# guenthermi/postgres-word2vec

Hardware: AMD Instinct MI355X
Metric: batched IVFADC kNN queries/sec (k=5) + recall@5, 3Mx300d (higher is better)
Workload: dtype f32; 1 GPU; IVFADC batch (ivfadc_batch_search generalised to nprobe), 3000000x300d, C=1000, m=12, K=1024, nprobe=10, k=5, batch=1024 queries per GPU, replicated index, queries sharded by rank; N=3000000, d=300, C=1000, m=12, K=1024, nprobe=10, k=5, batch_per_gpu=1024, parallelism=dp1, world_size=1, backend=none (single GPU), batches_in_flight=4

## Files before the change

postgres-word2vec_amd/csrc/fused5.h:

```cpp
#pragma once
#include <hip/hip_runtime.h>
#include <stdint.h>

#include "refine.h"
#include "coarse.h"
#include "scan_tail5.h"

namespace freddy {

static constexpr int SCAN5_G = 16;

__host__ __device__ __forceinline__ constexpr int filt5_bias(int p, int m) { return FILT5_VMAX + (p < 32768 - FILT5_VMAX * m ? 1 : 0); }
__device__ __forceinline__ uint32_t lane_byte4() {
  uint32_t x;
  asm volatile("v_mbcnt_lo_u32_b32 %0, -1, 0\n\tv_mbcnt_hi_u32_b32 %0, -1, %0\n\tv_lshlrev_b32 %0, 2, %0" : "=v"(x));
  return x;
}
typedef short s2v __attribute__((ext_vector_type(2)));
__device__ __forceinline__ uint32_t pk_add_i16(uint32_t x, uint32_t y) {
  return __builtin_bit_cast(uint32_t, __builtin_bit_cast(s2v, x) + __builtin_bit_cast(s2v, y));
}

template <int S, int QT>
__device__ __forceinline__ void query_codebook5_body(const float* __restrict__ queries, const float* __restrict__ cbT,
                                                     const float* __restrict__ cmax, float* __restrict__ qn,
                                                     float* __restrict__ qscale, uint32_t* __restrict__ qc,
                                                     int Q, int d, int m, int K, int bx, int by, unsigned char* smem,
                                                     uint32_t* __restrict__ qc8 = nullptr) {
  static_assert(QT == 16, "one 16-lane group per query");
  constexpr int SP = (S + 3) & ~3;
  float (*qs)[SP] = reinterpret_cast<float (*)[SP]>(smem);
  float* inv_s = reinterpret_cast<float*>(smem + QT * SP * 4);
  const int tid = threadIdx.x, p = bx, q0 = by * QT;
  static_assert(S <= 32 && SP % 4 == 0, "one k-step of v_mfma_f32_16x16x32_f16 covers a position");
  ch8v bh[8], bl[8];
  auto load_b = [&](int g) {
    const ch8v* src = reinterpret_cast<const ch8v*>(cbT) + ((size_t)p * 8 + g) * (CBF_GROUP_HALVES / 8) + (tid & 63);
#pragma unroll
    for (int t = 0; t < 8; ++t) { bh[t] = src[(size_t)t * 128]; bl[t] = src[(size_t)t * 128 + 64]; }
  };
  load_b((tid >> 6) * 2);
  const int ecb = reinterpret_cast<const int*>(cbT)[cbf_exp_offset(m) + p];
  for (int i = tid; i < QT * SP; i += 256) {
    const int qi = i / SP, j = i - qi * SP;
    qs[qi][j] = (j < S && q0 + qi < Q) ? queries[(size_t)(q0 + qi) * d + p * S + j] : 0.0f;
  }
  {
    const int qi = tid >> 4, pp = tid & 15, q = q0 + qi;
    float best = 0.0f;
    if (pp < m && q < Q) {
      float n2 = 0.0f;
      for (int j = 0; j < S; ++j) { const float v = queries[(size_t)q * d + pp * S + j]; n2 = __builtin_fmaf(v, v, n2); }
      const float nrm = __builtin_sqrtf(n2) * (1.0f + 1e-5f);
      if (p == 0) qn[(size_t)q * m + pp] = nrm;
      best = 2.0f * nrm * cmax[pp];
    }
#pragma unroll
    for (int o = 8; o > 0; o >>= 1) best = fmaxf(best, __shfl_xor(best, o, 64));
    if (pp == 0) {
      const float sc = q < Q ? best * (1.0f / (float)FILT5_VMAX) * (1.0f + 1e-6f) : 0.0f;
      inv_s[qi] = (sc > 0.0f && sc < 1e30f) ? 1.0f / sc : 0.0f;
      if (p == 0 && q < Q) qscale[q] = sc;
    }
  }
  {
    typedef float f4v __attribute__((ext_vector_type(4)));
    __syncthreads();
    const int wave = tid >> 6, lane = tid & 63, col = lane & 15, kq = lane >> 4;
    const int nq = (Q - q0 < QT) ? Q - q0 : QT;
    ch8v ah, al;
    int eq = 0;
    {
      f4v x0 = f4v{0.0f, 0.0f, 0.0f, 0.0f}, x1 = x0;
      if (8 * kq < SP) x0 = *reinterpret_cast<const f4v*>(&qs[col][8 * kq]);
      if (8 * kq + 4 < SP) x1 = *reinterpret_cast<const f4v*>(&qs[col][8 * kq + 4]);
      const float x[8] = {x0.x, x0.y, x0.z, x0.w, x1.x, x1.y, x1.z, x1.w};
      float am = 0.0f;
#pragma unroll
      for (int j = 0; j < 8; ++j) am = fmaxf(am, __builtin_fabsf(x[j]));
      am = fmaxf(am, __shfl_xor(am, 16, 64));
      am = fmaxf(am, __shfl_xor(am, 32, 64));
      if (am > 0.0f && am < 3e38f) { (void)__builtin_frexpf(am, &eq); eq = CBF_EXP - eq; }
#pragma unroll
      for (int j = 0; j < 8; ++j) {
        const float v = __builtin_ldexpf(x[j], eq);
        const _Float16 hh = (_Float16)v;
        ah[j] = hh;
        al[j] = (_Float16)(v - (float)hh);
      }
    }
    int unscale[4];
#pragma unroll
    for (int reg = 0; reg < 4; ++reg) unscale[reg] = -(__shfl(eq, 4 * kq + reg, 64) + ecb);
// ... 218 lines not shown
    };

    long long pt[8] = {0, 0, 0, 0, 0, 0, 0, 0}, pc = 0;
    auto tick = [&](int slot) { if constexpr (PROF) { const long long t = clock64(); pt[slot] += t - pc; pc = t; } };
    if constexpr (PROF) pc = clock64();
    int nq = (__builtin_amdgcn_readfirstlane(dsc[1]) + 7) >> 3;
    const int g0 = half * 8;
    int qid[8], nqid[8];
#pragma unroll
    for (int u = 0; u < 8; ++u) {
      qid[u] = __builtin_amdgcn_readfirstlane(dsc[24 + g0 + u]);
      nqid[u] = qid[u];
    }
    float rtv[RMAX];
    auto fetch_row_terms = [&](const int32_t* rc) {
      const int b0 = __builtin_amdgcn_readfirstlane(rc[3]), nbk = __builtin_amdgcn_readfirstlane(rc[4]);
#pragma unroll
      for (int r = 0; r < RMAX; ++r) {
        const int bl = r * NG + wave;
        rtv[r] = a.rterm[(size_t)(uint32_t)(b0 + (bl < nbk - 1 ? bl : nbk - 1)) * 64u + (uint32_t)lane];
      }
    };
    auto stash_row_terms = [&]() {
#pragma unroll
      for (int r = 0; r < RMAX; ++r) rt_s[(r * NG + wave) * 64 + lane] = rtv[r];
    };
    fetch_row_terms(dsc);
    stash_row_terms();
    issue(0, 0, qid, nq);
    issue(1, 1, qid, nq);
    emit(0, slab, nq);
    issue(0, 2, qid, nq);
    lds_barrier();
    for (;;) {
      const int nb = cur ^ 1;
      const int ngid = __builtin_amdgcn_readfirstlane(gidq[(ei + 1) & 1]);
      const bool have_next = ngid < n_work;
      int gid2 = 0;
      int next_nq = 0;
      int32_t rr0 = 0;
      uint32_t run0 = 0u, run1 = 0u;
#pragma unroll
      for (int j = 0; j < NP; ++j) {
        if (j == 1 && tid < REC_DW) {
          if (tid == 0) gidq[ei & 1] = gid2;
          dsc[nb * REC_DW + tid] = rr0;
          if (wave == 0 && lane == 6) dsc[nb * REC_DW + 6] = have_next ? 1 : -1;
        }
        if (j == NP - 3) {
          const int ncnt = have_next ? __builtin_amdgcn_readfirstlane(dsc[nb * REC_DW + 1]) : 0;
          next_nq = (ncnt + 7) >> 3;
#pragma unroll
          for (int u = 0; u < 8; ++u)
            nqid[u] = !have_next ? qid[u] : __builtin_amdgcn_readfirstlane(dsc[nb * REC_DW + 24 + g0 + u]);
        }
        const int set = (j + 1) & 1;
        if (j + 1 < NP) emit(set, slab + (uint32_t)((j + 1) & 1) * BUFB, nq);
        else emit(set, slab, next_nq);
        if (j + 3 < NP) issue(set, j + 3, qid, nq);
        else issue(set, j + 3 - NP, nqid, next_nq);
        if (j == 2) fetch_row_terms(dsc + (have_next ? nb : cur) * REC_DW);
        if (j == NP - 1 && a.tau_run) {
          const int32_t* rc = dsc + cur * REC_DW;
          const int cn = __builtin_amdgcn_readfirstlane(rc[1]);
          run0 = wave < cn ? a.tau_run[(uint32_t)rc[24 + wave]] : 0u;
          run1 = wave + NG < cn ? a.tau_run[(uint32_t)rc[24 + wave + NG]] : 0u;
        }
        if (j == 0 && tid < REC_DW && have_next) rr0 = a.records[(size_t)ngid * REC_DW + tid];
        if (j == 0 && tid == 0) {
          if (extra && (gidq[2] != 0 || !have_next)) {
            gid2 = 0x7fffffff;
          } else if (extra && __hip_atomic_load(a.elastic + EL_PENDING, FREDDY_RLX_AGENT) > 0) {
            gid2 = 0x7fffffff;
            gidq[2] = 1;
            __hip_atomic_fetch_add(a.elastic + EL_YIELDED, 1, FREDDY_RLX_AGENT);
          } else {
            gid2 = n_own + atomicAdd(a.work_counter, 1);
          }
        }
        tick(0);
        lds_barrier();
        tick(1);
      }
      if (!(a.fence & 4)) {
        const int32_t* rec = dsc + cur * REC_DW;
        const int cnt = __builtin_amdgcn_readfirstlane(rec[1]);
        const int i0 = wave, i1 = wave + NG;
        if (i0 < cnt) {
          uint32_t c0 = colmin[i0 * 64 + lane], c1 = colmin[i1 * 64 + lane];
          wave_sort32_x2(c0, c1);
          uint32_t t0 = __shfl(c0, a.Lt - 1, 64), t1 = __shfl(c1, a.Lt - 1, 64);
          if (lane == 0) {
            if (a.tau_run) {
              auto lower = [&](uint32_t t, int i, uint32_t inv) -> uint32_t {
                return running_bound5(a.tau_run, (uint32_t)rec[24 + i], t, __int_as_float(rec[144 + i]), __int_as_float(rec[160 + i]), inv);
              };
              t0 = lower(t0, i0, run0);
              if (i1 < cnt) t1 = lower(t1, i1, run1);
            }
            thr_s[i0] = a.keep_all ? 0x7f800000u : widen_threshold5(t0, __int_as_float(rec[56 + i0]));
            thr_s[i1] = a.keep_all ? 0x7f800000u : widen_threshold5(t1, __int_as_float(rec[56 + i1]));
          }
          colmin[i0 * 64 + lane] = 0xffffffffu;
          colmin[i1 * 64 + lane] = 0xffffffffu;
        }
      }
      lds_barrier();
      stash_row_terms();
      lds_barrier();
      tick(3);
      if constexpr (PROF) pt[7] += 1;
      if (!have_next) break;
      cur = nb;
      ++ei;
      nq = next_nq;
#pragma unroll
      for (int u = 0; u < 8; ++u) qid[u] = nqid[u];
    }
    if (ELASTIC && tid == 0) __hip_atomic_fetch_sub(a.elastic + EL_ACTIVE, 1, FREDDY_RLX_AGENT);
    if (PROF && a.prof && tid == 0) {
      for (int i = 0; i < 8; ++i) if (i != 2 && i != 4 && i != 5) a.prof[(size_t)blockIdx.x * 8 + i] = pt[i];
      a.prof[(size_t)blockIdx.x * 8 + 6] = wall_clock64();
    }
  } else {
    const int gw = wave - SPEC2_NB;
    uint32_t acc[G / 2][RMAX];
    uint32_t cwa[RMAX], cwb[RMAX];
    constexpr int NPRE = 2;
    uint32_t cpre[NPRE] = {};
    auto prefetch_first_codes = [&](const int32_t* rc) {
      const int b0 = __builtin_amdgcn_readfirstlane(rc[3]), nbk = __builtin_amdgcn_readfirstlane(rc[4]);
      const uint32_t l4 = lane_byte4();
#pragma unroll
      for (int r = 0; r < NPRE; ++r) {
        const int bl = r * NG + gw;
        const uint32_t blk = (uint32_t)(b0 + (bl < nbk - 1 ? bl : nbk - 1));
        const char* rowp = U8 ? reinterpret_cast<const char*>(a.packed8) + (size_t)(blk * (uint32_t)(M / 4)) * 256u
                              : reinterpret_cast<const char*>(a.packed) + (size_t)(blk * (uint32_t)(M / 2)) * 256u;
        cpre[r] = *reinterpret_cast<const uint32_t*>(rowp + l4);
      }
    };
    prefetch_first_codes(dsc);
    lds_barrier();
    long long gt[3] = {0, 0, 0}, gc = 0;
    auto gtick = [&](int slot) { if constexpr (PROF) { const long long t = clock64(); if (slot >= 0) gt[slot] += t - gc; gc = t; } };
    for (;;) {
      gtick(-1);
      const int32_t* rec = dsc + cur * REC_DW;
      const int cnt = __builtin_amdgcn_readfirstlane(rec[1]);
      const int chunk = __builtin_amdgcn_readfirstlane(rec[2]);
      const int blk0 = __builtin_amdgcn_readfirstlane(rec[3]);
      const int nblk = __builtin_amdgcn_readfirstlane(rec[4]);
      const int nrows = __builtin_amdgcn_readfirstlane(rec[5]);
      const int nq = (cnt + 7) >> 3;
      const int nb = cur ^ 1;
      const int rl_wave = (nblk - gw + NG - 1) / NG < 0 ? 0 : (nblk - gw + NG - 1) / NG;
      auto row_block = [&](int r) {
        const int bl = r * NG + gw;
        return (uint32_t)(blk0 + (bl < nblk - 1 ? bl : nblk - 1));
      };
      auto main_loop = [&](auto nqc, auto rlc) {
        constexpr int NQ = decltype(nqc)::value, RL = decltype(rlc)::value;
        auto load_codes = [&](uint32_t (&cw)[RMAX], int pair) {
          const uint32_t l4 = lane_byte4();
#pragma unroll
          for (int r = 0; r < RL; ++r) {
            const char* rowp = U8 ? reinterpret_cast<const char*>(a.packed8) + (size_t)((row_block(r) * (uint32_t)(M / 4) + (uint32_t)(pair >> 1)) * 256u)
                                  : reinterpret_cast<const char*>(a.packed) + (size_t)((row_block(r) * (uint32_t)(M / 2) + (uint32_t)pair) * 256u);
            cw[r] = *reinterpret_cast<const uint32_t*>(rowp + l4);
          }
        };
        auto gather = [&](const uint32_t (&cw)[RMAX], int j) {
          constexpr int DEPTH = NQ == 1 ? 4 : 2;
          u4 va[DEPTH][2][NQ];
          uint32_t bb = (uint32_t)(j & 1) * BUFB;
          asm volatile("" : "+s"(bb));
          auto issue_row = [&](int r) {
            const uint32_t a0 = (U8 ? ((j & 1) ? ((cw[r] >> 12) & 0xff0u) : ((cw[r] << 4) & 0xff0u)) : ((cw[r] << 4) & 0x3ff0u)) + bb;
            const uint32_t a1 = (U8 ? ((j & 1) ? ((cw[r] >> 20) & 0xff0u) : ((cw[r] >> 4) & 0xff0u)) : ((cw[r] >> 12) & 0x3ff0u)) + bb;
#pragma unroll
            for (int q = 0; q < NQ; ++q) va[r % DEPTH][0][q] = *reinterpret_cast<const u4*>(slab + a0 + (uint32_t)q * HALFB);
#pragma unroll
            for (int q = 0; q < NQ; ++q) va[r % DEPTH][1][q] = *reinterpret_cast<const u4*>(slab + a1 + POSB + (uint32_t)q * HALFB);
          };
#pragma unroll
          for (int r = 0; r < DEPTH - 1; ++r) if (r < RL) issue_row(r);
#pragma unroll
          for (int r = 0; r < RL; ++r) {
            if (r + DEPTH - 1 < RL) issue_row(r + DEPTH - 1);
#pragma unroll
            for (int q = 0; q < NQ; ++q) {
              const u4 x = va[r % DEPTH][0][q], y = va[r % DEPTH][1][q];
              acc[q * 4 + 0][r] = acc[q * 4 + 0][r] + x.x + y.x;
              acc[q * 4 + 1][r] = acc[q * 4 + 1][r] + x.y + y.y;
              acc[q * 4 + 2][r] = acc[q * 4 + 2][r] + x.z + y.z;
              acc[q * 4 + 3][r] = acc[q * 4 + 3][r] + x.w + y.w;
            }
            if (r + 1 < RL) __builtin_amdgcn_sched_barrier(0);
          }
        };
#pragma unroll
        for (int h = 0; h < G / 2; ++h)
#pragma unroll
          for (int r = 0; r < RMAX; ++r) acc[h][r] = 0u;
        load_codes(cwa, 0);
#pragma unroll
        for (int r = 0; r < NPRE; ++r) if (r < RL) cwa[r] = cpre[r];
        load_codes(cwb, 1);
#pragma unroll
        for (int j = 0; j < NP; ++j) {
          if (!(a.fence & 2)) {
            if (j & 1) gather(cwb, j); else gather(cwa, j);
          }
          __builtin_amdgcn_sched_barrier(0);
          if (j + 2 < NP && !(a.fence & 64)) {
            if (j & 1) load_codes(cwb, j + 2); else load_codes(cwa, j + 2);
          }
          if (j + 1 < NP) lds_barrier();
        }
      };
      dispatch_nq_rl(nq, rl_wave, main_loop);
#define SCAN_TAIL5_FENCE a.fence
#define SCAN_TAIL5_PART 1
#include "scan_tail5.inc"
      gtick(0);
#define SCAN_TAIL5_PART 2
#include "scan_tail5.inc"
      gtick(1);
      lds_barrier();
      lds_barrier();
      gtick(-1);
#define SCAN_TAIL5_PART 3
#include "scan_tail5.inc"
#undef SCAN_TAIL5_FENCE
      gtick(2);
      const int next_ok = __builtin_amdgcn_readfirstlane(dsc[nb * REC_DW + 6]);
      if (next_ok > 0) prefetch_first_codes(dsc + nb * REC_DW);
      lds_barrier();
      if (next_ok < 0) break;
      cur = nb;
    }
    if (PROF && a.prof && gw == 0 && lane == 0) {
      a.prof[(size_t)blockIdx.x * 8 + 2] = gt[0];
      a.prof[(size_t)blockIdx.x * 8 + 4] = gt[1];
      a.prof[(size_t)blockIdx.x * 8 + 5] = gt[2];
    }
  }
}

template <int M, bool FULLK, bool CAND, bool PROF = false, bool U8 = false>
__global__ __launch_bounds__(SPEC2_T) void ivf_filter5_kernel(FilterArgs a) {
  ivf_filter5_body<M, FULLK, CAND, PROF, U8, false>(a);
}
template <int M, bool FULLK, bool CAND, bool U8 = false>
__global__ __launch_bounds__(SPEC2_T) void ivf_filter5_elastic_kernel(FilterArgs a) {
  ivf_filter5_body<M, FULLK, CAND, false, U8, true>(a);
}

}
```

postgres-word2vec_amd/csrc/ivfadc.hip:

```cpp
#include "internal.h"

#include <functional>

#include "kernels.h"
#include "scan_common.h"
#include "fused3.h"
#include "fused5.h"
#include "fused8.h"
#include "one.h"
#include "sparse5.h"
#include "coarse.h"
#include "multi.h"
#include "io_kernels.h"
#include "bigk.h"
#include "ivf_host.h"
#include "query_ids.h"

static void (*scan_kernel(bool m12, int V, bool floor))(ScanArgs) {
  void (*k)(ScanArgs) = nullptr;
  if (floor) return V != 16 ? nullptr : m12 ? &adc_scan_kernel<12, 16, true> : &adc_scan_kernel<0, 16, true>;
  with_V(V, [&](auto v) { k = m12 ? &adc_scan_kernel<12, decltype(v)::value> : &adc_scan_kernel<0, decltype(v)::value>; });
  return k;
}
static void (*filter_kernel(bool whole, bool u8, bool k1024, bool counts_rows, bool prof, bool elastic = false))(FilterArgs) {
// ... 165 lines not shown
    else if (r.approx)
      hipLaunchKernelGGL(coarse_approx_kernel, dim3(Cpad / 128, (Q + COARSE_TQ - 1) / COARSE_TQ), dim3(256),
                         (size_t)(COARSE_TQ * (ix->dp + 4) + 128) * sizeof(float), s, r.d_q, ix->coarseP, ix->cn2,
                         ws->w_distT.as<float>(), ws->w_qn2.as<float>(), Q, Cpad, d, ix->dp, za, tile_min, C);
    else if (r.tiled)
      hipLaunchKernelGGL((coarse_tile_kernel<2, 16>), dim3(Cpad / 32, (Q + 63) / 64), dim3(256), 0, s, r.d_q, ix->coarseT,
                         ws->w_distT.as<float>(), Q, Cpad, d, za);
    else if (small_zero)
      hipLaunchKernelGGL((coarse_small_kernel<50>), dim3(Cpad / 64, Q), dim3(64), 0, s, r.d_q, ix->coarseT, ws->w_distT.as<float>(), Q, Cpad, d, za);
    else
      hipLaunchKernelGGL((coarse_dist_kernel<16>), dim3(Cpad / WG, (Q + 15) / 16), dim3(WG), (size_t)d * 16 * sizeof(float), s, r.d_q,
                         ix->coarseT, ws->w_distT.as<float>(), Q, Cpad, d);
  });
  HIP_TRY(hipGetLastError());
  return 0;
}

static int ivf_plan(IvfRun& r, PlanArgs& pa) {
  Workspace* ws = r.ws;
  freddy_gpu_index* ix = r.ix;
  hipStream_t s = r.s;
  const int C = ix->C, W = r.W;
  pa = plan_items(r, C);
  pa.dist = ws->w_distT.as<float>(); pa.active = r.active; pa.list_off = ix->list_off;
  pa.used = ws->w_used.as<uint32_t>(); pa.Cpad = ix->Cpad; pa.used_words = (C + 31) / 32;
  pa.cell_count = r.fused ? ws->w_cellcnt.as<int32_t>() : nullptr;
  pa.cell_items = r.fused ? ws->w_sorted.as<int32_t>() : nullptr; pa.cell_cap = r.n_active;
  pa.cell_limit = r.cell_limit;
  const int n_items = r.n_active * W;
  if (r.fused && !(r.zeroed && r.first())) {
    HIP_TRY(hipMemsetAsync(ws->w_cellcnt.p, 0, sizeof(int32_t) * (size_t)C * 2, s));
    HIP_TRY(hipMemsetAsync(ws->w_surv_cnt.p, 0, sizeof(int32_t) * surv_regions(r, (size_t)n_items), s));
  }
  const int PV = pick_V(2 * W);
  const size_t plan_lds = (size_t)(64 + 64 * PV) * sizeof(u64) + (size_t)W * 8;
  if (r.approx) {
    Plan2Args g;
    g.p = pa; g.queries = r.d_q; g.coarse = ix->coarse; g.qn2 = ws->w_qn2.as<float>(); g.item_dist = pa.item_dist;
    g.violations = ix->viol; g.cmax = ix->cmax; g.d = ix->d; g.refine_all = (ix->tune.check_brackets & 2) ? 1 : 0; g.prof = nullptr;
    g.tmin = (r.first() && ix->Cpad > COARSE_MAX_CPAD && ws->w_tmin.p) ? ws->w_tmin.as<float>() : nullptr;
    timed_launch(ix, s, "probe_plan", [&] {
      if (ix->Cpad <= COARSE_MAX_CPAD && r.share > 1) hipLaunchKernelGGL((probe_plan2_kernel<0, false, 1>), dim3(r.n_active), dim3(64), 0, s, g);
      else if (ix->Cpad <= COARSE_MAX_CPAD) hipLaunchKernelGGL((probe_plan2_kernel<0, false>), dim3(r.n_active), dim3(64 * PLAN2_NW), 0, s, g);
      else hipLaunchKernelGGL((probe_plan2_kernel<0, true>), dim3(r.n_active), dim3(64 * PLAN2_NW), 0, s, g);
    });
  } else
  timed_launch(ix, s, "probe_plan", [&] {
    with_V(PV, [&](auto v) { hipLaunchKernelGGL((probe_plan_kernel<decltype(v)::value>), dim3(r.n_active), dim3(64), plan_lds, s, pa); });
  });
  HIP_TRY(hipGetLastError());
  if (!(r.zeroed && r.first())) HIP_TRY(hipMemsetAsync(ws->w_cand.p, 0, sizeof(int32_t) * 2 * r.Q, s));
  return 0;
}

int ivf_work_table(IvfRun& r, WorkTable& wt) {
  Workspace* ws = r.ws;
  freddy_gpu_index* ix = r.ix;
  hipStream_t s = r.s;
  const int n_items = r.n_active * r.W;
  wt = work_counters(ws, ((size_t)n_items / MULTI_G + (size_t)ix->C + 1) * r.upi);
  int32_t* base = ws->w_groups.as<int32_t>();
  wt.group_cell = base; wt.group_first = base + wt.max_groups; wt.group_cnt = base + 2 * wt.max_groups;
  const int sparse_max = r.scan_kernel != 5 ? 0
                         : ix->tune.sparse_items < 0 ? -ix->tune.sparse_items
                         : sparse_by_itself(ix->n_cus, n_items, ix->C) ? ix->tune.sparse_items : 0;
  wt.sp_cap = sparse_max > 0 ? (size_t)n_items * r.upi : 0;
  wt.sp_cell = base + 3 * wt.max_groups; wt.sp_first = wt.sp_cell + wt.sp_cap; wt.sp_chunk = wt.sp_first + wt.sp_cap;
  timed_launch(ix, s, "work_table", [&] {
    hipLaunchKernelGGL(work_table_kernel, dim3(1), dim3(1024), 0, s, ws->w_cellcnt.as<int32_t>(), ix->C, r.n_active, r.scan_kernel == 5 ? SCAN5_G : r.scan_kernel == 2 ? MULTI_G : SPEC2_G, ix->blk_off,
                       wt.group_cell, wt.group_first, wt.group_cnt, wt.n_groups, r.scan_kernel == 5 ? 2 : 0,
                       sparse_max, wt.sp_cell, wt.sp_first, wt.sp_chunk, wt.n_sparse, sparse_max >= 2 ? 1 : 0);
  });
  wt.sp_pairs = sparse_max >= 2;
  HIP_TRY(hipGetLastError());
  if (!(r.zeroed && r.first())) HIP_TRY(hipMemsetAsync(wt.work_counter, 0, 2 * sizeof(int32_t), s));
  return 0;
}

static int scan_prof_buffer(freddy_gpu_index* ix, Workspace* ws, long long** prof, uint32_t* fence = nullptr) {
  *prof = nullptr;
#ifdef FREDDY_LAB
  if (fence) *fence = (uint32_t)ix->tune.scan_fence;
  if (!ix->tune.scan_prof) return 0;
  if (ws->w_prof.ensure(sizeof(long long) * 8 * 1024)) return fail(FREDDY_E_NOMEM, "profile buffer");
  *prof = ws->w_prof.as<long long>();
#endif
  (void)ix; (void)ws; (void)fence;
  return 0;
}

#ifdef FREDDY_LAB
static int scan_prof_print(freddy_gpu_index* ix, hipStream_t s, const long long* prof, unsigned n_persist) {
  std::vector<long long> h(8 * (size_t)n_persist);
  HIP_TRY(hipStreamSynchronize(s));
  HIP_TRY(hipMemcpy(h.data(), prof, sizeof(long long) * h.size(), hipMemcpyDeviceToHost));
  double sum[8] = {0}; long long mx_end = 0, mn_end = -1; double ent = 0;
  for (unsigned b = 0; b < n_persist; ++b) {
    for (int i = 0; i < 6; ++i) sum[i] += (double)h[b * 8 + i];
    ent += (double)h[b * 8 + 7];
    mx_end = std::max(mx_end, h[b * 8 + 6]);
    mn_end = mn_end < 0 ? h[b * 8 + 6] : std::min(mn_end, h[b * 8 + 6]);
  }
  fprintf(stderr, "[scan prof] wgs=%u entries=%.0f  builder cycles/entry: builds=%.0f barrier-wait=%.0f tail=%.0f | gatherer wave 0 (fused5.h): main=%.0f colmin=%.0f S2=%.0f | workgroups ran dry over %.1f us\n",
          n_persist, ent, sum[0] / ent, sum[1] / ent, sum[3] / ent, sum[2] / ent, sum[4] / ent, sum[5] / ent, (mx_end - mn_end) / 100.0);
  (void)ix;
  return 0;
}
static int filter_prof_print(freddy_gpu_index* ix, hipStream_t s, const FilterArgs& fl, bool whole, unsigned n_persist) {
  if (!fl.prof || fl.cand_count || !(whole || fl.K == 1024)) return 0;
  if (!whole) return scan_prof_print(ix, s, fl.prof, n_persist);
  std::vector<long long> h(8 * (size_t)n_persist);
  HIP_TRY(hipStreamSynchronize(s));
  HIP_TRY(hipMemcpy(h.data(), fl.prof, sizeof(long long) * h.size(), hipMemcpyDeviceToHost));
  double sum[8] = {0}, life_max = 0, life_min = 1e30;
  for (unsigned b = 0; b < n_persist; ++b) {
    for (int i = 0; i < 8; ++i) sum[i] += (double)h[b * 8 + i];
    life_max = std::max(life_max, (double)h[b * 8 + 7]); life_min = std::min(life_min, (double)h[b * 8 + 7]);
  }
  int32_t ng = 0;
  HIP_TRY(hipMemcpy(&ng, fl.n_groups, 4, hipMemcpyDeviceToHost));
  const double e = std::max(1, ng);
  fprintf(stderr, "[scan8 prof] wgs=%u entries=%d  gatherer wave 0 cycles/entry (slots 0-5): gather=%.0f B1=%.0f colmin=%.0f B2=%.0f S1=%.0f B3+S2+B4=%.0f | per workgroup: prologue (slot 6) %.0f, stages (0-5) %.0f, life (slot 7) mean %.0f min %.0f max %.0f\n",
          n_persist, ng, sum[0] / e, sum[1] / e, sum[2] / e, sum[3] / e, sum[4] / e, sum[5] / e, sum[6] / n_persist,
          (sum[0] + sum[1] + sum[2] + sum[3] + sum[4] + sum[5]) / n_persist, sum[7] / n_persist, life_min, life_max);
  return 0;
}
#endif

int ivf_scan_filter(IvfRun& r, const PlanArgs& pa, const WorkTable& wt) {
  Workspace* ws = r.ws;
  freddy_gpu_index* ix = r.ix;
  hipStream_t s = r.s;
  const int K = ix->K;
  const QueryTable qt = query_table(ws, ix, r.Q);
  const unsigned n_own = filter_scan_own(ix->n_cus, r.share, ix->tune.reserve_cus, wt.max_groups);
  const bool u8 = ix->packed8 && ix->tune.codes_u8 != 0 && ix->K <= 256;
  const bool whole = u8 && qt.qc8;
  bool elastic = ix->tune.scan_elastic > 0 && r.share > 1 && !r.records_ready && !whole && ix->elastic != nullptr;
#ifdef FREDDY_LAB
  if (ix->tune.scan_prof) elastic = false;
#endif
  const int cap = filter_scan_cap(ix->n_cus, ix->tune.scan_elastic_reserve, ix->tune.reserve_cus, r.share);
  const unsigned n_persist = filter_scan_persist(elastic, n_own, cap, wt.max_groups);
  if (!r.records_ready) {
    if (ws->w_records.ensure(sizeof(int32_t) * REC_DW * wt.max_groups)) return fail(FREDDY_E_NOMEM, "workspace allocation failed");
    RecordArgs ra;
    ra.group_cell = wt.group_cell; ra.group_first = wt.group_first; ra.group_cnt = wt.group_cnt; ra.n_groups = wt.n_groups;
    ra.sorted_item = ws->w_sorted.as<int32_t>(); ra.item_query = pa.item_query; ra.blk_off = ix->blk_off; ra.list_off = ix->list_off;
    ra.item_dist = pa.item_dist; ra.qn = qt.qn; ra.qscale = qt.qscale; ra.pmax = ix->pmax;
    ra.records = ws->w_records.as<int32_t>(); ra.sentinel = r.sentinel;
    ra.elastic = elastic ? ix->elastic : nullptr; ra.n_announce = (int)n_own;
    timed_launch(ix, s, "entry_records", [&] {
      hipLaunchKernelGGL((entry_record5_kernel<12>), dim3((unsigned)((wt.max_groups + 3) / 4)), dim3(256), 0, s, ra);
    });
    HIP_TRY(hipGetLastError());
  }
  FilterArgs fl;
  fl.qc = qt.qc; fl.qc8 = qt.qc8; fl.rterm = ix->rterm; fl.records = ws->w_records.as<int32_t>(); fl.n_groups = wt.n_groups;
  fl.work_counter = wt.work_counter; fl.packed = ix->packed; fl.surv = ws->w_surv.as<u64>(); fl.surv_count = ws->w_surv_cnt.as<int32_t>();
  fl.cand_count = rows_counter(r);
  fl.K = K; fl.L = r.L; fl.Lt = r.Lt; fl.upi = r.upi; fl.sentinel = r.sentinel; fl.keep_all = (ix->tune.check_brackets & 1) ? 1 : 0; fl.fence = 0;
  fl.tau_run = r.running_bound ? ws->w_cand.as<uint32_t>() + r.Q : nullptr;
  if (int rc = scan_prof_buffer(ix, ws, &fl.prof, &fl.fence)) return rc;
  fl.elastic = elastic ? ix->elastic : nullptr; fl.n_own = (int)n_own; fl.cap = cap; fl.elastic_yield = ix->tune.scan_elastic;
  const size_t desc_off = whole ? (size_t)scan8_slab_bytes(12) : (size_t)4 * SCAN5_G * 2 * K;
  const size_t flds = desc_off + 4096 + 64 + (2 * REC_DW + 4) * sizeof(int32_t) + 4096 * sizeof(float);
  fl.desc_offset = (uint32_t)desc_off;
  fl.packed8 = u8 ? ix->packed8 : nullptr;
  const auto filter = filter_kernel(whole, u8, K == 1024, fl.cand_count != nullptr, fl.prof != nullptr, elastic);
  if (!filter) return fail(FREDDY_E_ARG, "internal: no filter scan for this shape");
  timed_launch(ix, s, "ivf_filter", [&] { hipLaunchKernelGGL(filter, dim3(n_persist), dim3(SPEC2_T), flds, s, fl); });
  HIP_TRY(hipGetLastError());
  if (wt.sp_cap > 0) {
    SparseArgs sp;
    sp.qc = qt.qc; sp.qscale = qt.qscale; sp.qn = qt.qn; sp.pmax = ix->pmax; sp.rterm = ix->rterm; sp.packed = ix->packed;
    sp.blk_off = ix->blk_off; sp.list_off = ix->list_off; sp.sorted_item = ws->w_sorted.as<int32_t>(); sp.item_query = pa.item_query;
    sp.item_dist = pa.item_dist; sp.sp_cell = wt.sp_cell; sp.sp_first = wt.sp_first; sp.sp_chunk = wt.sp_chunk;
    sp.n_units = wt.n_sparse; sp.work_counter = wt.sp_counter; sp.surv = fl.surv; sp.surv_count = fl.surv_count; sp.packed8 = fl.packed8;
    sp.cand_count = fl.cand_count; sp.K = K; sp.L = r.L; sp.Lt = r.Lt; sp.upi = r.upi; sp.sentinel = r.sentinel; sp.keep_all = fl.keep_all; sp.tau_run = fl.tau_run;
    const unsigned sp_grid = sparse_grid(ix->n_cus, r.share, ix->tune.reserve_cus, wt.sp_cap, wt.sp_pairs);
    const auto sparse = sparse_kernel(wt.sp_pairs, u8, fl.cand_count != nullptr);
    timed_launch(ix, s, "sparse_items", [&] { hipLaunchKernelGGL(sparse, dim3(sp_grid), dim3(256), 0, s, sp); });
    HIP_TRY(hipGetLastError());
  }
#ifdef FREDDY_LAB
  if (int rc = filter_prof_print(ix, s, fl, whole, n_persist)) return rc;
#endif

  MergeRefineArgs mr;
  mr.surv = fl.surv; mr.surv_count = fl.surv_count; mr.active = r.active; mr.round_rows = pa.round_rows;
  mr.item_cell = pa.item_cell; mr.queries = r.d_q; mr.coarse = ix->coarse; mr.cbR = ix->cbR;
  mr.qn = qt.qn; mr.pmax = ix->pmax; mr.qscale5 = qt.qscale; mr.packed = ix->packed; mr.pos = ix->pos; mr.blk_cell = ix->blk_cell;
  mr.cand_count = fl.cand_count; mr.violations = ix->viol; mr.out_ids = r.d_out_ids; mr.out_dist = r.d_out_dist;
  mr.found = ws->w_found.as<int32_t>(); mr.next_active = r.next; mr.n_next = ws->w_cnt.as<int32_t>();
  mr.status = r.d_status;
  mr.n_active = r.n_active; mr.W = r.W; mr.upi = r.upi; mr.L = r.L; mr.k = r.k; mr.found_rule = r.found_rule;
  mr.first_round = r.first() ? 1 : 0; mr.K = K; mr.d = ix->d; mr.sentinel = r.sentinel;
  mr.refine_all = (ix->tune.check_brackets & 1) ? 1 : 0; mr.fence = 0;
  mr.slices = 0; mr.part = nullptr;
  if (r.merge_slices > 0) {
    const int SL = r.merge_slices;
    if (ws->w_part.ensure(sizeof(u64) * (size_t)r.n_active * SL * r.L)) return fail(FREDDY_E_NOMEM, "workspace allocation failed");
    mr.slices = SL; mr.part = ws->w_part.as<u64>(); mr.W = r.W / SL; mr.n_active = r.n_active * SL;
    timed_launch(ix, s, "merge_refine", [&] {
      hipLaunchKernelGGL((merge_refine_kernel<25, 12, 12, true, true>), dim3(r.n_active * SL), dim3(768), 0, s, mr);
    });
    HIP_TRY(hipGetLastError());
    return launch_merge(ix, s, merge_args_flat(mr.part, r.n_active, SL, r.L, r.k, r.sentinel, nullptr, r.d_out_ids, r.d_out_dist));
  }
  timed_launch(ix, s, "merge_refine", [&] {
    const bool many_regions = (size_t)r.W * r.upi * FUSED_NW > 256;
    if (!many_regions && r.share > 1)
      hipLaunchKernelGGL((merge_refine_kernel<25, 12, 1>), dim3(r.n_active), dim3(64), 0, s, mr);
    else if (many_regions && r.n_active <= 256)
      hipLaunchKernelGGL((merge_refine_kernel<25, 12, 12, true>), dim3(r.n_active), dim3(768), 0, s, mr);
    else if (many_regions)
      hipLaunchKernelGGL((merge_refine_kernel<25, 12, 4, true>), dim3(r.n_active), dim3(256), 0, s, mr);
    else
      hipLaunchKernelGGL((merge_refine_kernel<25, 12, 4>), dim3(r.n_active), dim3(256), 0, s, mr);
  });
  HIP_TRY(hipGetLastError());
  return 0;
}

static int launch_merge_surv(const IvfRun& r, const PlanArgs& pa, const u64* surv, const int32_t* surv_count, const int32_t* cand_count) {
  MergeSurvArgs ms;
  ms.surv = surv; ms.surv_count = surv_count; ms.active = r.active; ms.round_rows = pa.round_rows;
  ms.cand_count = cand_count; ms.out_ids = r.d_out_ids; ms.out_dist = r.d_out_dist;
  ms.found = r.ws->w_found.as<int32_t>(); ms.next_active = r.next; ms.n_next = r.ws->w_cnt.as<int32_t>();
  ms.status = r.d_status;
  ms.n_active = r.n_active; ms.W = r.W; ms.upi = r.upi; ms.L = r.L; ms.k = r.k; ms.found_rule = r.found_rule;
  ms.first_round = r.first() ? 1 : 0; ms.sentinel = r.sentinel;
  timed_launch(r.ix, r.s, "merge_surv", [&] { hipLaunchKernelGGL(merge_surv_kernel, dim3(r.n_active), dim3(64), 0, r.s, ms); });
  HIP_TRY(hipGetLastError());
  return 0;
}

static int ivf_scan_exact(IvfRun& r, const PlanArgs& pa, const WorkTable& wt) {
  Workspace* ws = r.ws;
  freddy_gpu_index* ix = r.ix;
  hipStream_t s = r.s;
  const int K = ix->K;
  FusedArgs fa;
  fa.resid = nullptr; fa.item_query = pa.item_query; fa.queries = r.d_q; fa.coarse = ix->coarse;
  fa.sorted_item = ws->w_sorted.as<int32_t>(); fa.group_cell = wt.group_cell; fa.group_first = wt.group_first;
  fa.group_cnt = wt.group_cnt; fa.n_groups = wt.n_groups; fa.work_counter = wt.work_counter;
// ... 482 lines not shown
```

postgres-word2vec_amd/csrc/scan_tail5.inc:

```
#if SCAN_TAIL5_PART == 1
float base[RMAX];
const int last_blk = nrows > 0 ? (nrows - 1) >> 6 : -1;
const int rs2 = (last_blk >= 0 && (last_blk % NG) == gw && (nrows & 63)) ? last_blk / NG : -1;
const bool live_lane = lane < (nrows & 63);
{
#pragma unroll
  for (int r = 0; r < RMAX; ++r) {
    base[r] = rt_s[(r * NG + gw) * 64 + lane];
    if (r >= rl_wave || (r == rs2 && !live_lane)) base[r] = __uint_as_float(0x7f800000u);
  }
}
#pragma unroll
for (int h = 0; h < G / 2; ++h)
#pragma unroll
  for (int r = 0; r < RMAX; ++r) acc[h][r] ^= 0x80008000u;
#elif SCAN_TAIL5_PART == 2
auto sval = [&](int g, int r, float sc) -> float {
  const uint32_t w = acc[g >> 1][r];
  const int v = (g & 1) ? ((int32_t)w >> 16) : ((int32_t)(w << 16) >> 16);
  return __builtin_fmaf(sc, (float)v, base[r]);
};
const int gi = lane & 15;
const float p_sc = __int_as_float(rec[128 + gi]);
uint32_t live8 = 0u;
#pragma unroll
for (int r = 0; r < RMAX; ++r)
  if (r < rl_wave && !(r == rs2 && !live_lane)) live8 |= 1u << r;
float best[G];
uint32_t sec16[G / 2];
uint32_t apack[2] = {0u, 0u};
#pragma unroll
for (int g = 0; g < G; ++g) best[g] = __uint_as_float(0x7f800000u);
#pragma unroll
for (int i = 0; i < G / 2; ++i) sec16[i] = 0x7f807f80u;
if (!(SCAN_TAIL5_FENCE & 4)) {
#pragma unroll
  for (int g = 0; g < G; ++g) {
    if (g < cnt) {
      const float sc = __int_as_float(__builtin_amdgcn_readlane(__float_as_int(p_sc), g));
      float b1 = __uint_as_float(0x7f800000u), b2 = __uint_as_float(0x7f800000u);
      uint32_t ar = 0u;
#pragma unroll
      for (int r = 0; r < RMAX; ++r) {
        const float sv = sval(g, r, sc);
        b2 = __builtin_amdgcn_fmed3f(b1, b2, sv);
        ar = sv < b1 ? (uint32_t)r : ar;
        b1 = fminf(b1, sv);
      }
      best[g] = b1;
      {
        const uint32_t bb = __float_as_uint(b2);
        const uint32_t dn = ((bb >> 31) ? bb + 0xffffu : bb) >> 16;
        sec16[g >> 1] = (g & 1) ? ((sec16[g >> 1] & 0x0000ffffu) | (dn << 16)) : ((sec16[g >> 1] & 0xffff0000u) | dn);
      }
      asm volatile("" : "+v"(ar));
      apack[g >> 3] |= ar << (3 * (g & 7));
      if (rl_wave > 0) atomicMin(colmin + g * 64 + lane, float_key(b1));
    }
  }
}
#elif SCAN_TAIL5_PART == 3
if (!(SCAN_TAIL5_FENCE & 4)) {
  const float p_thr = __uint_as_float(thr_s[gi]);
  const int p_it = rec[8 + gi];
  const float p_shift = __int_as_float(rec[72 + gi]);
  const float p_off = __int_as_float(rec[40 + gi]);
  const uint32_t p_lo = (uint32_t)rec[88 + gi], p_hi = (uint32_t)rec[104 + gi];
  const int p_q = rec[24 + gi];
  const int p_reg = (p_it * a.upi + chunk) * NG + gw;
  int cntv = 0;
#pragma unroll
  for (int g = 0; g < G; ++g) {
    if (g < cnt) {
      const float thr = __int_as_float(__builtin_amdgcn_readlane(__float_as_int(p_thr), g));
      const float off = __int_as_float(__builtin_amdgcn_readlane(__float_as_int(p_off), g));
      const float shift = __int_as_float(__builtin_amdgcn_readlane(__float_as_int(p_shift), g));
      const uint32_t region = (uint32_t)__builtin_amdgcn_readlane(p_reg, g);
      u64* dst = a.surv + (size_t)region * (size_t)(RMAX * 64);
      int run = 0;
      if constexpr (!CAND) {
       const float second = __uint_as_float((g & 1) ? (sec16[g >> 1] & 0xffff0000u) : (sec16[g >> 1] << 16));
       const u64 multi = __ballot(!(second > thr));
       if (__builtin_expect(multi == 0ull, 1)) {
        const bool pass = !(best[g] > thr);
        const u64 mask = __ballot(pass);
        if (pass) {
          const uint32_t r = (apack[g >> 3] >> (3 * (g & 7))) & 7u;
          const float dlo = fmaxf(0.0f, (best[g] + off) - shift);
          const uint32_t loc = ((uint32_t)(blk0 + gw) + r * (uint32_t)NG) * 64u + (uint32_t)lane;
          dst[lanes_below(mask)] = surv_key5(dlo, loc);
        }
        run = __popcll(mask);
       } else {
        const float sc = __int_as_float(__builtin_amdgcn_readlane(__float_as_int(p_sc), g));
        uint32_t m8 = 0u;
#pragma unroll
        for (int r = RMAX - 1; r >= 0; --r) m8 = m8 + m8 + (!(sval(g, r, sc) > thr) ? 1u : 0u);
        m8 &= live8;
        if ((SCAN_TAIL5_FENCE & 128) == 0 && __ballot(m8 != 0u) != 0ull) {
#pragma unroll
          for (int r = 0; r < RMAX; ++r) {
            const bool pass = (m8 >> r) & 1u;
            const u64 mask = __ballot(pass);
            if (mask != 0ull) {
              if (pass) {
                const float dlo = fmaxf(0.0f, (sval(g, r, sc) + off) - shift);
                const uint32_t loc = (uint32_t)(blk0 + r * NG + gw) * 64u + (uint32_t)lane;
                dst[run + lanes_below(mask)] = surv_key5(dlo, loc);
              }
              run += __popcll(mask);
            }
          }
        }
       }
      } else {
        const uint32_t lo_b = (uint32_t)__builtin_amdgcn_readlane((int)p_lo, g);
        const uint32_t hi_b = (uint32_t)__builtin_amdgcn_readlane((int)p_hi, g);
        const float sc = __int_as_float(__builtin_amdgcn_readlane(__float_as_int(p_sc), g));
        int accepted = 0;
#pragma unroll
        for (int r = 0; r < RMAX; ++r) {
          if (r >= rl_wave) break;
          const float sv = sval(g, r, sc);
          const uint32_t sb = __float_as_uint(sv + off);
          const bool live = (live8 >> r) & 1u;
          accepted += __popcll(__ballot(live && sb < lo_b));
          const bool amb = sb >= lo_b && sb < hi_b;
          const bool pass = live && (!(sv > thr) || amb);
          const u64 mask = __ballot(pass);
          if (mask != 0ull) {
            if (pass) {
              const float dlo = fmaxf(0.0f, __uint_as_float(sb) - shift);
              const uint32_t loc = ((uint32_t)(blk0 + r * NG + gw) * 64u + (uint32_t)lane) | (amb ? 0x80000000u : 0u);
              dst[run + lanes_below(mask)] = surv_key5(dlo, loc);
            }
            run += __popcll(mask);
          }
        }
        if (lane == 0 && accepted) atomicAdd(a.cand_count + __builtin_amdgcn_readlane(p_q, g), accepted);
      }
      asm("v_writelane_b32 %0, %1, %2" : "+v"(cntv) : "s"(run), "i"(g));
    }
  }
  if (lane < cnt) a.surv_count[(uint32_t)p_reg] = cntv;
}
#else
#error "SCAN_TAIL5_PART: 1, 2 or 3"
#endif
#undef SCAN_TAIL5_PART
```

Before: 12.37 million queries/s.

## Split per-entry threshold and scan tail into two halves of eight groups

The builder waves compute per-query thresholds in two phases, and the second half runs only when an entry holds more than eight queries. The gatherer tail (row minima and survivor emission) is split the same way, with barriers between halves, so the first eight groups can proceed once their thresholds are ready. Entries with eight or fewer queries skip the second half's work and barriers. This adds extra barriers and more macro-included code, and it extends the profiling buffer to record the tail waits.

```diff
diff --git a/postgres-word2vec_amd/csrc/fused5.h b/postgres-word2vec_amd/csrc/fused5.h
--- a/postgres-word2vec_amd/csrc/fused5.h
+++ b/postgres-word2vec_amd/csrc/fused5.h
@@ -9,6 +9,7 @@
 namespace freddy {
 
 static constexpr int SCAN5_G = 16;
+static constexpr int SCAN5_PROF_WGS = 1024;
 
 __host__ __device__ __forceinline__ constexpr int filt5_bias(int p, int m) { return FILT5_VMAX + (p < 32768 - FILT5_VMAX * m ? 1 : 0); }
 __device__ __forceinline__ uint32_t lane_byte4() {
@@ -393,30 +394,22 @@
         lds_barrier();
         tick(1);
       }
-      if (!(a.fence & 4)) {
-        const int32_t* rec = dsc + cur * REC_DW;
-        const int cnt = __builtin_amdgcn_readfirstlane(rec[1]);
-        const int i0 = wave, i1 = wave + NG;
-        if (i0 < cnt) {
-          uint32_t c0 = colmin[i0 * 64 + lane], c1 = colmin[i1 * 64 + lane];
-          wave_sort32_x2(c0, c1);
-          uint32_t t0 = __shfl(c0, a.Lt - 1, 64), t1 = __shfl(c1, a.Lt - 1, 64);
-          if (lane == 0) {
-            if (a.tau_run) {
-              auto lower = [&](uint32_t t, int i, uint32_t inv) -> uint32_t {
-                return running_bound5(a.tau_run, (uint32_t)rec[24 + i], t, __int_as_float(rec[144 + i]), __int_as_float(rec[160 + i]), inv);
-              };
-              t0 = lower(t0, i0, run0);
-              if (i1 < cnt) t1 = lower(t1, i1, run1);
-            }
-            thr_s[i0] = a.keep_all ? 0x7f800000u : widen_threshold5(t0, __int_as_float(rec[56 + i0]));
-            thr_s[i1] = a.keep_all ? 0x7f800000u : widen_threshold5(t1, __int_as_float(rec[56 + i1]));
-          }
-          colmin[i0 * 64 + lane] = 0xffffffffu;
-          colmin[i1 * 64 + lane] = 0xffffffffu;
-        }
-      }
+      const int32_t* rec_t = dsc + cur * REC_DW;
+      const int cnt_t = __builtin_amdgcn_readfirstlane(rec_t[1]);
+      auto threshold = [&](int i, uint32_t run) {
+        if (i < cnt_t && !(a.fence & 4)) {
+          const uint32_t c = wave_sort32(colmin[i * 64 + lane]);
+          const uint32_t t = __shfl(c, a.Lt - 1, 64);
+          if (lane == 0) thr_s[i] = filter_threshold5(a, rec_t, i, t, run);
+          colmin[i * 64 + lane] = 0xffffffffu;
+        }
+      };
+      threshold(wave, run0);
       lds_barrier();
+      if (cnt_t > 8) {
+        threshold(wave + NG, run1);
+        lds_barrier();
+      }
       stash_row_terms();
       lds_barrier();
       tick(3);
@@ -453,7 +446,7 @@
     };
     prefetch_first_codes(dsc);
     lds_barrier();
-    long long gt[3] = {0, 0, 0}, gc = 0;
+    long long gt[8] = {0, 0, 0, 0, 0, 0, 0, 0}, gc = 0;
     auto gtick = [&](int slot) { if constexpr (PROF) { const long long t = clock64(); if (slot >= 0) gt[slot] += t - gc; gc = t; } };
     for (;;) {
       gtick(-1);
@@ -536,18 +529,43 @@
 #include "scan_tail5.inc"
       gtick(0);
 #define SCAN_TAIL5_PART 2
+#define SCAN_TAIL5_G0 0
+#define SCAN_TAIL5_G1 8
 #include "scan_tail5.inc"
       gtick(1);
       lds_barrier();
+      gtick(3);
+      if (cnt > 8) {
+#define SCAN_TAIL5_PART 2
+#define SCAN_TAIL5_G0 8
+#define SCAN_TAIL5_G1 16
+#include "scan_tail5.inc"
+      }
+      gtick(1);
       lds_barrier();
-      gtick(-1);
+      gtick(4);
 #define SCAN_TAIL5_PART 3
+#define SCAN_TAIL5_G0 0
+#define SCAN_TAIL5_G1 8
+#include "scan_tail5.inc"
+      gtick(2);
+      if (cnt > 8) {
+        lds_barrier();
+        gtick(5);
+#define SCAN_TAIL5_PART 3
+#define SCAN_TAIL5_G0 8
+#define SCAN_TAIL5_G1 16
+#include "scan_tail5.inc"
+      }
+#define SCAN_TAIL5_PART 4
 #include "scan_tail5.inc"
 #undef SCAN_TAIL5_FENCE
       gtick(2);
       const int next_ok = __builtin_amdgcn_readfirstlane(dsc[nb * REC_DW + 6]);
       if (next_ok > 0) prefetch_first_codes(dsc + nb * REC_DW);
       lds_barrier();
+      gtick(6);
+      if constexpr (PROF) gt[7] += cnt > 8 ? 1 : 0;
       if (next_ok < 0) break;
       cur = nb;
     }
@@ -555,6 +573,8 @@
       a.prof[(size_t)blockIdx.x * 8 + 2] = gt[0];
       a.prof[(size_t)blockIdx.x * 8 + 4] = gt[1];
       a.prof[(size_t)blockIdx.x * 8 + 5] = gt[2];
+      long long* p2 = a.prof + ((size_t)SCAN5_PROF_WGS + blockIdx.x) * 8;
+      for (int i = 0; i < 5; ++i) p2[i] = gt[3 + i];
     }
   }
 }
diff --git a/postgres-word2vec_amd/csrc/ivfadc.hip b/postgres-word2vec_amd/csrc/ivfadc.hip
--- a/postgres-word2vec_amd/csrc/ivfadc.hip
+++ b/postgres-word2vec_amd/csrc/ivfadc.hip
@@ -271,7 +271,8 @@
 #ifdef FREDDY_LAB
   if (fence) *fence = (uint32_t)ix->tune.scan_fence;
   if (!ix->tune.scan_prof) return 0;
-  if (ws->w_prof.ensure(sizeof(long long) * 8 * 1024)) return fail(FREDDY_E_NOMEM, "profile buffer");
+  if (ws->w_prof.ensure(sizeof(long long) * 16 * SCAN5_PROF_WGS))
+    return fail(FREDDY_E_NOMEM, "profile buffer");
   *prof = ws->w_prof.as<long long>();
 #endif
   (void)ix; (void)ws; (void)fence;
@@ -279,8 +280,8 @@
 }
 
 #ifdef FREDDY_LAB
-static int scan_prof_print(freddy_gpu_index* ix, hipStream_t s, const long long* prof, unsigned n_persist) {
-  std::vector<long long> h(8 * (size_t)n_persist);
+static int scan_prof_print(freddy_gpu_index* ix, hipStream_t s, const long long* prof, unsigned n_persist, bool tail_waits = false) {
+  std::vector<long long> h(tail_waits ? 8 * ((size_t)SCAN5_PROF_WGS + n_persist) : 8 * (size_t)n_persist);
   HIP_TRY(hipStreamSynchronize(s));
   HIP_TRY(hipMemcpy(h.data(), prof, sizeof(long long) * h.size(), hipMemcpyDeviceToHost));
   double sum[8] = {0}; long long mx_end = 0, mn_end = -1; double ent = 0;
@@ -292,12 +293,19 @@
   }
   fprintf(stderr, "[scan prof] wgs=%u entries=%.0f  builder cycles/entry: builds=%.0f barrier-wait=%.0f tail=%.0f | gatherer wave 0 (fused5.h): main=%.0f colmin=%.0f S2=%.0f | workgroups ran dry over %.1f us\n",
           n_persist, ent, sum[0] / ent, sum[1] / ent, sum[3] / ent, sum[2] / ent, sum[4] / ent, sum[5] / ent, (mx_end - mn_end) / 100.0);
+  if (tail_waits) {
+    double w[5] = {0};
+    for (unsigned b = 0; b < n_persist; ++b)
+      for (int i = 0; i < 5; ++i) w[i] += (double)h[((size_t)SCAN5_PROF_WGS + b) * 8 + i];
+    fprintf(stderr, "[scan prof] gatherer wave 0 waits, cycles/entry: T1=%.0f T2=%.0f T3=%.0f last=%.0f | entry total=%.0f | entries of more than 8 items: %.0f\n",
+            w[0] / ent, w[1] / ent, w[2] / ent, w[3] / ent, (sum[2] + sum[4] + sum[5] + w[0] + w[1] + w[2] + w[3]) / ent, w[4]);
+  }
   (void)ix;
   return 0;
 }
 static int filter_prof_print(freddy_gpu_index* ix, hipStream_t s, const FilterArgs& fl, bool whole, unsigned n_persist) {
   if (!fl.prof || fl.cand_count || !(whole || fl.K == 1024)) return 0;
-  if (!whole) return scan_prof_print(ix, s, fl.prof, n_persist);
+  if (!whole) return scan_prof_print(ix, s, fl.prof, n_persist, true);
   std::vector<long long> h(8 * (size_t)n_persist);
   HIP_TRY(hipStreamSynchronize(s));
   HIP_TRY(hipMemcpy(h.data(), fl.prof, sizeof(long long) * h.size(), hipMemcpyDeviceToHost));
@@ -351,6 +359,7 @@
   fl.K = K; fl.L = r.L; fl.Lt = r.Lt; fl.upi = r.upi; fl.sentinel = r.sentinel; fl.keep_all = (ix->tune.check_brackets & 1) ? 1 : 0; fl.fence = 0;
   fl.tau_run = r.running_bound ? ws->w_cand.as<uint32_t>() + r.Q : nullptr;
   if (int rc = scan_prof_buffer(ix, ws, &fl.prof, &fl.fence)) return rc;
+  if (n_persist > (unsigned)SCAN5_PROF_WGS) fl.prof = nullptr;
   fl.elastic = elastic ? ix->elastic : nullptr; fl.n_own = (int)n_own; fl.cap = cap; fl.elastic_yield = ix->tune.scan_elastic;
   const size_t desc_off = whole ? (size_t)scan8_slab_bytes(12) : (size_t)4 * SCAN5_G * 2 * K;
   const size_t flds = desc_off + 4096 + 64 + (2 * REC_DW + 4) * sizeof(int32_t) + 4096 * sizeof(float);
diff --git a/postgres-word2vec_amd/csrc/scan_tail5.inc b/postgres-word2vec_amd/csrc/scan_tail5.inc
--- a/postgres-word2vec_amd/csrc/scan_tail5.inc
+++ b/postgres-word2vec_amd/csrc/scan_tail5.inc
@@ -15,6 +15,11 @@
 #pragma unroll
   for (int r = 0; r < RMAX; ++r) acc[h][r] ^= 0x80008000u;
 #elif SCAN_TAIL5_PART == 2
+#ifndef SCAN_TAIL5_G0
+#define SCAN_TAIL5_G0 0
+#define SCAN_TAIL5_G1 G
+#endif
+#if SCAN_TAIL5_G0 == 0
 auto sval = [&](int g, int r, float sc) -> float {
   const uint32_t w = acc[g >> 1][r];
   const int v = (g & 1) ? ((int32_t)w >> 16) : ((int32_t)(w << 16) >> 16);
@@ -33,9 +38,10 @@
 for (int g = 0; g < G; ++g) best[g] = __uint_as_float(0x7f800000u);
 #pragma unroll
 for (int i = 0; i < G / 2; ++i) sec16[i] = 0x7f807f80u;
+#endif
 if (!(SCAN_TAIL5_FENCE & 4)) {
 #pragma unroll
-  for (int g = 0; g < G; ++g) {
+  for (int g = SCAN_TAIL5_G0; g < SCAN_TAIL5_G1; ++g) {
     if (g < cnt) {
       const float sc = __int_as_float(__builtin_amdgcn_readlane(__float_as_int(p_sc), g));
       float b1 = __uint_as_float(0x7f800000u), b2 = __uint_as_float(0x7f800000u);
@@ -59,7 +65,15 @@
     }
   }
 }
+#undef SCAN_TAIL5_G0
+#undef SCAN_TAIL5_G1
 #elif SCAN_TAIL5_PART == 3
+#ifndef SCAN_TAIL5_G0
+#define SCAN_TAIL5_G0 0
+#define SCAN_TAIL5_G1 G
+#define SCAN_TAIL5_WHOLE
+#endif
+#ifdef SCAN_TAIL5_WHOLE
 if (!(SCAN_TAIL5_FENCE & 4)) {
   const float p_thr = __uint_as_float(thr_s[gi]);
   const int p_it = rec[8 + gi];
@@ -69,8 +83,25 @@
   const int p_q = rec[24 + gi];
   const int p_reg = (p_it * a.upi + chunk) * NG + gw;
   int cntv = 0;
+#else
+#if SCAN_TAIL5_G0 == 0
+float p_shift = 0.0f, p_off = 0.0f;
+uint32_t p_lo = 0u, p_hi = 0u;
+int p_q = 0, p_reg = 0;
+int cntv = 0;
+#endif
+if (!(SCAN_TAIL5_FENCE & 4)) {
+  const float p_thr = __uint_as_float(*reinterpret_cast<const uint32_t*>(reinterpret_cast<const char*>(thr_s) + (lane_byte4() & 60u)));
+#if SCAN_TAIL5_G0 == 0
+  p_shift = __int_as_float(rec[72 + gi]);
+  p_off = __int_as_float(rec[40 + gi]);
+  p_lo = (uint32_t)rec[88 + gi]; p_hi = (uint32_t)rec[104 + gi];
+  p_q = rec[24 + gi];
+  p_reg = (rec[8 + gi] * a.upi + chunk) * NG + gw;
+#endif
+#endif
 #pragma unroll
-  for (int g = 0; g < G; ++g) {
+  for (int g = SCAN_TAIL5_G0; g < SCAN_TAIL5_G1; ++g) {
     if (g < cnt) {
       const float thr = __int_as_float(__builtin_amdgcn_readlane(__float_as_int(p_thr), g));
       const float off = __int_as_float(__builtin_amdgcn_readlane(__float_as_int(p_off), g));
@@ -142,9 +173,18 @@
       asm("v_writelane_b32 %0, %1, %2" : "+v"(cntv) : "s"(run), "i"(g));
     }
   }
+#ifdef SCAN_TAIL5_WHOLE
+  if (lane < cnt) a.surv_count[(uint32_t)p_reg] = cntv;
+#endif
+}
+#undef SCAN_TAIL5_G0
+#undef SCAN_TAIL5_G1
+#undef SCAN_TAIL5_WHOLE
+#elif SCAN_TAIL5_PART == 4
+if (!(SCAN_TAIL5_FENCE & 4)) {
   if (lane < cnt) a.surv_count[(uint32_t)p_reg] = cntv;
 }
 #else
-#error "SCAN_TAIL5_PART: 1, 2 or 3"
+#error "SCAN_TAIL5_PART: 1 .. 4"
 #endif
 #undef SCAN_TAIL5_PART
```

New measurement: 12.63 million queries/s, median of 6. +2.1%, better.
